# facebookresearch/CODD

Hardware: AMD Instinct MI355X
Metric: frames/sec full CODD forward @960x540 (whole job) (higher is better)
Workload: dtype f32 (split-bf16 MFMA operands, f32 accumulate; HITNet + context network + Fusion exact f32); 1 GPU; full CODD (HITNetMF + Motion/RAFT3D iters=16 + Fusion) 960x540 padded to 960x576, max_disp=320, one video per GPU, steady-state frames (idx>=1), synthetic stereo sequence, random-init weights; conv_precision=split, hip_graph=True, frames_per_gpu=304, prewarm_frames=150, side_streams=True, library=codd_amd/csrc/libcodd_hip.so, full=False

## Files before the change

codd_amd/_abi.py:

```python
import ctypes as C
import os

from . import build as _build

c_float_p = C.POINTER(C.c_float)


class View(C.Structure):
    _fields_ = [("ptr", C.c_void_p), ("ctot", C.c_int), ("coff", C.c_int)]


class XsView(C.Structure):
    _fields_ = [("ptr", C.c_void_p), ("c8", C.c_int), ("hp", C.c_int), ("wp", C.c_int), ("bt", C.c_int),
                ("bl", C.c_int), ("o8", C.c_int), ("terms", C.c_int)]


class ConvParams(C.Structure):
    _fields_ = [
        ("in0", View), ("in1", View), ("C0", C.c_int), ("C1", C.c_int),
        ("B", C.c_int), ("Hin", C.c_int), ("Win", C.c_int),
        ("wpacked", C.c_void_p), ("bias", C.c_void_p),
        ("res1", View), ("res2", View), ("post", View),
        ("out", C.c_void_p), ("out_ctot", C.c_int), ("out_coff", C.c_int),
        ("Cout", C.c_int), ("Hout", C.c_int), ("Wout", C.c_int),
# ... 8 lines not shown
    ]


ACT = dict(none=0, lrelu=1, relu=2, sigmoid=3, tanh=4, mish=5, relu_ch0=6)




class RollParams(C.Structure):
    _fields_ = [("in0", View), ("in1", View), ("C0", C.c_int), ("C1", C.c_int),
                ("B", C.c_int), ("H", C.c_int), ("W", C.c_int), ("C", C.c_int), ("mode", C.c_int),
                ("wA", C.c_void_p), ("bA", C.c_void_p), ("wB", C.c_void_p), ("bB", C.c_void_p),
                ("actA", C.c_int), ("actB", C.c_int), ("residual", C.c_int),
                ("out", C.c_void_p), ("out_ctot", C.c_int), ("out_coff", C.c_int), ("cout_store", C.c_int),
                ("rh", C.c_int)]


_i, _f, _p, _ll = C.c_int, C.c_float, C.c_void_p, C.c_longlong

SIGNATURES = {
    "codd_abi_version": (_i, []),
    "codd_conv2d": (_i, [C.POINTER(ConvParams), _p]),
    "codd_conv2d_check": (_i, [C.POINTER(ConvParams)]),
    "codd_conv2d_multi": (_i, [C.POINTER(ConvParams), _i, _p]),
    "codd_roll_packed_size": (_ll, [_i, _i, _i]),
    "codd_roll_pack_weights": (_i, [_p, _p, _i, _i, _i, _i, _p]),
    "codd_conv_roll": (_i, [C.POINTER(RollParams), _p]),
    "codd_conv2d_packed_size": (_ll, [_i] * 6),
    "codd_conv2d_pack_weights": (_i, [_p, _p, _i, _i, _i, _i, _i, _i, _p]),
    "codd_tile_costvol_argmin": (_i, [_p, _p, _i, _i, _i, _i, _i, _i, _p, _i, _i, _p, _i, _i, _i, _p]),
    "codd_tile_warp_cost": (_i, [_p, _p, _i, _i, _i, _i, View, View, _i, _p, _p, _p]),
    "codd_hyp_upsample": (_i, [View, _i, _i, _i, _f, _p, _i, _i, _p]),
    "codd_hyp_select": (_i, [_p, View, View, _i, _i, _i, _p, _i, _i, _p]),
    "codd_instnorm": (_i, [_p, _i, _i, _i, _p, _p, _i, _p, _p]),
    "codd_instnorm_xs": (_i, [_p, _i, _i, _i, _i, _p, _p, _i, _i, _p, XsView, _p]),
    "codd_conv2d_pack_weights_ex": (_i, [_p, _p, _i, _i, _i, _i, _i, _i, _ll, _ll, _f, _p]),
    "codd_allpairs_corr": (_i, [_p, _p, _i, _i, _i, _i, _p, _p, _p, _p, _p, _p]),
    "codd_allpairs_corr_scratch": (_ll, [_i, _i, _i, _i]),
    "codd_avgpool2": (_i, [_p, _i, _i, _i, _p, _p]),
    "codd_induced_flow": (_i, [_p, _p, _i, _i, _i, _f, _f, _f, _f, _p, _p]),
    "codd_context_split": (_i, [_p, _i, _i, _p, _p, _p]),
    "codd_se3_identity": (_i, [_p, _ll, _p]),
    "codd_corr_lookup": (_i, [_p, _p, _p, _p, _p, _i, _i, _i, _i, _p, _p]),
    "codd_raft_geometry": (_i, [_p, _p, _p, _i, _i, _i, _f, _f, _f, _f, _p, _p, _p]),
    "codd_se3_gn_step": (_i, [_p, _p, _i, _p, _p, _p, _p, _i, _i, _i, _f, _f, _f, _f, _i, _f, _f, _p, _p]),
    "codd_se3_gn_scratch": (_ll, [_i, _i, _i, _i]),
    "codd_set_option": (_i, [_i, _i]),
    "codd_get_option": (_i, [_i]),
    "codd_se3_gn_step_heads": (_i, [_p, XsView, _p, _p, _p, _p, _i, _i, _i, _f, _f, _f, _f, _i, _f, _f, _p, _p, _p]),
    "codd_cvx_upsample": (_i, [_p, _p, _i, _i, _i, _i, _i, _p, _p]),
    "codd_cvx_upsample_se3_weight": (_i, [_p, _p, _p, _i, _i, _i, _p, _p, _p]),
    "codd_disp_to_depth": (_i, [_p, _ll, _f, _p, _p]),
    "codd_subsample": (_i, [_p, _i, _i, _i, _i, _i, _i, _p, _p]),
    "codd_splat": (_i, [_p, _p, _i, _i, _i, _i, _i, _p, _i, _p, _i, _i, _i, _i, _i, _f, _f, _f, _f, _f, _f,
                        _p, _p, _p, _p]),
    "codd_splat_scratch": (_ll, [_i, _i, _i, _f]),
    "codd_resize_bilinear": (_i, [_p, _i, _i, _i, _i, _i, _i, _i, _p, _i, _i, _i, _i, _p]),
    "codd_resize_bilinear_add": (_i, [_p, _i, _i, _i, _i, _i, _i, _i, _p, _i, _i, _i, _i, _p, _p]),
    "codd_add_relu": (_i, [_p, _p, _ll, _i, _p, _p]),
    "codd_copy_many": (_i, [_p, _p, _p, _i, _p]),
    "codd_copy": (_i, [_p, _p, _ll, _p]),
    "codd_timestamp": (_i, [_p, _p]),
    "codd_gru_gate_zr": (_i, [_p, _p, _p, _p, _p, _p, _i, _i, _p, _p, _p]),
    "codd_gru_gate_q": (_i, [_p, _p, _p, _p, _p, _p, _p, _i, _i, _p, _p]),
    "codd_gru_gate_zr_xs": (_i, [_p, _p, _p, _p, _p, _p, _i, _i, _i, _p, XsView, _p]),
    "codd_gru_gate_q_xs": (_i, [_p, _p, _p, _p, _p, _p, _p, _i, _i, _i, _p, XsView, _p]),
# ... 98 lines not shown
```

codd_amd/csrc/stereo.hip:

```cpp
#include "common.h"
#include <stdlib.h>

#define CV_TPB 16
__global__ __launch_bounds__(256) void costvol_argmin_kernel(const float* __restrict__ L, const float* __restrict__ R,
                                                             int C, int Ht, int Wt, int Wr, int D, float* cost,
                                                             int cost_ctot, int cost_coff, float* disp, int disp_ctot,
                                                             int disp_coff, int zero_dxdy) {
  extern __shared__ float sm[];
  const int tid = threadIdx.x, lane = tid & 63, wave = tid >> 6;
  const int xt0 = blockIdx.x * CV_TPB, y = blockIdx.y, b = blockIdx.z;
  const int win = D + 4 * (CV_TPB - 1);
  const int base = 4 * xt0 - (D - 1);
  float* rl = sm;
  float* ll = sm + C * win;
  const float* Rb = R + ((size_t)b * C * Ht + y) * Wr;
  for (int e = tid; e < C * win; e += 256) {
    const int c = e / win, i = e - c * win, gx = base + i;
    rl[e] = (gx >= 0 && gx < Wr) ? Rb[(size_t)c * Ht * Wr + gx] : 0.f;
  }
  const float* Lb = L + ((size_t)b * C * Ht + y) * Wt;
  for (int e = tid; e < C * CV_TPB; e += 256) {
    const int c = e / CV_TPB, i = e - c * CV_TPB, gx = xt0 + i;
    ll[e] = gx < Wt ? Lb[(size_t)c * Ht * Wt + gx] : 0.f;
  }
// ... 105 lines not shown
  }
}

extern "C" int codd_tile_costvol_argmin(const float* L, const float* R, int B, int C, int Ht, int Wt, int Wr, int D,
                                        float* cost, int cost_ctot, int cost_coff, float* disp, int disp_ctot,
                                        int disp_coff, int zero_dxdy, void* stream) {
  if (!L || !R || !cost || !disp || B < 1 || C < 1 || D < 1 || Ht < 1 || Wt < 1) return CODD_EINVAL;
  hipStream_t st = (hipStream_t)stream;
  if ((D & 3) == 0) {
    int tpb = 16;
    for (;; tpb >>= 1) {
      const int win = D + 4 * (tpb - 1);
      const size_t lds = (size_t)(C * win + C * tpb) * sizeof(float);
      if (lds > 64 * 1024) { if (tpb == 16) return CODD_EUNSUPPORTED; continue; }
      dim3 grid(cdiv(Wt, tpb), Ht, B);
#define CV_LAUNCH(T) costvol_argmin4_kernel<T><<<grid, 256, lds, st>>>(L, R, C, Ht, Wt, Wr, D, cost, cost_ctot, cost_coff, disp, disp_ctot, disp_coff, zero_dxdy)
      if (tpb == 64) CV_LAUNCH(64); else if (tpb == 32) CV_LAUNCH(32); else CV_LAUNCH(16);
#undef CV_LAUNCH
      break;
    }
    CODD_LAUNCH_CHECK();
    return CODD_OK;
  }
  const int win = D + 4 * (CV_TPB - 1);
  size_t lds = (size_t)(C * win + C * CV_TPB) * sizeof(float);
  if (lds > 64 * 1024) return CODD_EUNSUPPORTED;
  dim3 grid(cdiv(Wt, CV_TPB), Ht, B);
  costvol_argmin_kernel<<<grid, 256, lds, st>>>(L, R, C, Ht, Wt, Wr, D, cost, cost_ctot, cost_coff,
                                                disp, disp_ctot, disp_coff, zero_dxdy);
  CODD_LAUNCH_CHECK();
  return CODD_OK;
}

template <bool STAGE>
__global__ __launch_bounds__(256) void tile_warp_kernel(const float* __restrict__ fl, const float* __restrict__ fr,
                                                        int C, int Ht, int Wt, codd_view h0, codd_view h1, int nhyp,
                                                        float* out0, float* out1) {
  extern __shared__ __attribute__((aligned(16))) float srow[];
  const int txr = blockIdx.x * blockDim.x + threadIdx.x;
  const int yy = blockIdx.y;
  const int b = blockIdx.z;
  if (!STAGE && txr >= Wt) return;
  const bool live = txr < Wt;
  const int tx = live ? txr : Wt - 1;
  const int ty = yy >> 2, iy = yy & 3;
  const int H = 4 * Ht, W = 4 * Wt;
  if (STAGE) {
    const float4* src = (const float4*)(fr + (size_t)b * C * H * W + (size_t)yy * W);
    const int w4 = W >> 2, chw4 = (H * W) >> 2;
    for (int c = 0; c < C; ++c)
      for (int x4 = threadIdx.x; x4 < w4; x4 += blockDim.x) ((float4*)srow)[c * w4 + x4] = src[(size_t)c * chw4 + x4];
    __syncthreads();
  }
  const size_t thw = (size_t)Ht * Wt, tpix = (size_t)ty * Wt + tx;
  const float* flb = fl + (size_t)b * C * H * W + (size_t)yy * W + 4 * tx;
  const float* frb = fr + (size_t)b * C * H * W + (size_t)yy * W;
  const size_t chw = (size_t)H * W;

  int f0[2][4];
  float a[2][4];
  unsigned okm[2] = {0u, 0u};
#pragma unroll
  for (int hsel = 0; hsel < 2; ++hsel) {
    const codd_view hv = (hsel && nhyp == 2) ? h1 : h0;
    const float* hp = hv.ptr + ((size_t)b * hv.ctot + hv.coff) * thw + tpix;
    const float d = hp[0], dx = hp[thw], dy = hp[2 * thw];
#pragma unroll
    for (int ix = 0; ix < 4; ++ix) {
      const float delta = d + (ix - 1.5f) * dx + (iy - 1.5f) * dy;
      const float xs = (float)(4 * tx + ix) - delta;
      const float fl0 = floorf(xs);
      a[hsel][ix] = xs - fl0;
      f0[hsel][ix] = (int)fminf(fmaxf(fl0, -4.f), (float)W + 4.f);
#pragma unroll
      for (int q = 0; q < 4; ++q)
        if ((unsigned)(f0[hsel][ix] - 1 + q) < (unsigned)W) okm[hsel] |= 1u << (ix * 4 + q);
    }
  }
  float fea[4] = {0.f, 0.f, 0.f, 0.f};
  float cv[2][3][4] = {{{0.f}}};
#pragma unroll 2
  for (int c = 0; c < C; ++c) {
    const float4 l4 = *(const float4*)(flb + c * chw);
    const float lv[4] = {l4.x, l4.y, l4.z, l4.w};
    const float* rr = frb + c * chw;
    float t[2][4][4];
#pragma unroll
    for (int hsel = 0; hsel < 2; ++hsel) {
      if (hsel < nhyp) {
#pragma unroll
        for (int ix = 0; ix < 4; ++ix)
#pragma unroll
          for (int q = 0; q < 4; ++q) {
            const int xi = min(max(f0[hsel][ix] - 1 + q, 0), W - 1);
            t[hsel][ix][q] = STAGE ? srow[c * W + xi] : rr[xi];
          }
      }
    }
#pragma unroll
    for (int ix = 0; ix < 4; ++ix) fea[ix] += fabsf(lv[ix]);
#pragma unroll
    for (int hsel = 0; hsel < 2; ++hsel) {
      if (hsel < nhyp) {
#pragma unroll
        for (int ix = 0; ix < 4; ++ix) {
          float tq[4];
#pragma unroll
          for (int q = 0; q < 4; ++q) tq[q] = (okm[hsel] >> (ix * 4 + q)) & 1u ? t[hsel][ix][q] : 0.f;
          const float w1 = a[hsel][ix], w0 = 1.f - a[hsel][ix];
          cv[hsel][0][ix] += fabsf(lv[ix] - (w0 * tq[2] + w1 * tq[3]));
          cv[hsel][1][ix] += fabsf(lv[ix] - (w0 * tq[1] + w1 * tq[2]));
          cv[hsel][2][ix] += fabsf(lv[ix] - (w0 * tq[0] + w1 * tq[1]));
        }
      }
    }
  }
  if (!live) return;
#pragma unroll
  for (int ix = 0; ix < 4; ++ix) {
    const int ch = iy * 4 + ix;
    const size_t o = (size_t)b * 64 * thw + tpix;
    out0[o + (size_t)ch * thw] = fea[ix];
    if (nhyp == 2) out1[o + (size_t)ch * thw] = fea[ix];
#pragma unroll
    for (int k = 0; k < 3; ++k) {
      out0[o + (size_t)(16 + k * 16 + ch) * thw] = cv[0][k][ix];
      if (nhyp == 2) out1[o + (size_t)(16 + k * 16 + ch) * thw] = cv[1][k][ix];
    }
  }
}

extern "C" int codd_tile_warp_cost(const float* fl, const float* fr, int B, int C, int Ht, int Wt, codd_view hyp0,
                                   codd_view hyp1, int nhyp, float* out0, float* out1, void* stream) {
  if (!fl || !fr || !hyp0.ptr || !out0 || nhyp < 1 || nhyp > 2 || (nhyp == 2 && (!hyp1.ptr || !out1)))
    return CODD_EINVAL;
  const size_t lds = (size_t)C * 4 * Wt * sizeof(float);
  if (lds <= 96 * 1024 && ((uintptr_t)fr & 15) == 0) {
    if (lds > 64 * 1024 &&
        hipFuncSetAttribute((const void*)tile_warp_kernel<true>, hipFuncAttributeMaxDynamicSharedMemorySize, (int)lds) != hipSuccess)
      return CODD_EUNSUPPORTED;
    const int bx = Wt > 128 ? 256 : (Wt > 64 ? 128 : 64);
    dim3 grid(cdiv(Wt, bx), 4 * Ht, B);
    tile_warp_kernel<true><<<grid, bx, lds, (hipStream_t)stream>>>(fl, fr, C, Ht, Wt, hyp0, hyp1, nhyp, out0, out1);
    CODD_LAUNCH_CHECK();
    return CODD_OK;
  }
  const int bx = 64;
  dim3 grid(cdiv(Wt, bx), 4 * Ht, B);
  tile_warp_kernel<false><<<grid, bx, 0, (hipStream_t)stream>>>(fl, fr, C, Ht, Wt, hyp0, hyp1, nhyp, out0, out1);
  CODD_LAUNCH_CHECK();
  return CODD_OK;
}

__global__ void hyp_upsample_kernel(codd_view in, int h, int w, float scale, float* out, int out_ctot, int out_coff,
                                    long long total) {
  long long e = (long long)blockIdx.x * blockDim.x + threadIdx.x;
  if (e >= total) return;
  const int W2 = 2 * w, H2 = 2 * h;
  const int x = (int)(e % W2);
  long long t = e / W2;
  const int y = (int)(t % H2); t /= H2;
  const int c = (int)(t % 16);
  const int b = (int)(t / 16);
  const size_t hw = (size_t)h * w;
  const float* ip = in.ptr + ((size_t)b * in.ctot + in.coff) * hw + (size_t)(y >> 1) * w + (x >> 1);
  float v;
  if (c == 0) {
    const float cx = (x & 1) ? 0.5f : -0.5f, cy = (y & 1) ? 0.5f : -0.5f;
    v = (ip[0] + cx * ip[hw] + cy * ip[2 * hw]) * scale;
  } else {
    v = ip[(size_t)c * hw];
  }
  out[((size_t)b * out_ctot + out_coff + c) * (size_t)(4 * hw) + (size_t)y * W2 + x] = v;
}

extern "C" int codd_hyp_upsample(codd_view in, int B, int h, int w, float scale, float* out, int out_ctot,
                                 int out_coff, void* stream) {
  if (!in.ptr || !out) return CODD_EINVAL;
  long long total = (long long)B * 16 * 4 * h * w;
  hyp_upsample_kernel<<<cdiv(total, 256), 256, 0, (hipStream_t)stream>>>(in, h, w, scale, out, out_ctot, out_coff,
                                                                         total);
  CODD_LAUNCH_CHECK();
  return CODD_OK;
}

__global__ void hyp_select_kernel(const float* __restrict__ upd, codd_view cur, codd_view prev, int hw, float* out,
                                  int out_ctot, int out_coff, long long total) {
  long long e = (long long)blockIdx.x * blockDim.x + threadIdx.x;
  if (e >= total) return;
  const int pix = (int)(e % hw);
  long long t = e / hw;
  const int c = (int)(t % 16);
  const int b = (int)(t / 16);
  const float* u = upd + (size_t)b * 34 * hw + pix;
  const bool sel_cur = u[hw] > u[0];
  float v;
  if (sel_cur) v = cur.ptr[((size_t)b * cur.ctot + cur.coff + c) * hw + pix] + u[(size_t)(18 + c) * hw];
  else v = prev.ptr[((size_t)b * prev.ctot + prev.coff + c) * hw + pix] + u[(size_t)(2 + c) * hw];
  if (c == 0) v = fmaxf(v, 0.f);
  out[((size_t)b * out_ctot + out_coff + c) * hw + pix] = v;
}

extern "C" int codd_hyp_select(const float* upd, codd_view cur, codd_view prev, int B, int h, int w, float* out,
                               int out_ctot, int out_coff, void* stream) {
  if (!upd || !cur.ptr || !prev.ptr || !out) return CODD_EINVAL;
  long long total = (long long)B * 16 * h * w;
  hyp_select_kernel<<<cdiv(total, 256), 256, 0, (hipStream_t)stream>>>(upd, cur, prev, h * w, out, out_ctot, out_coff,
                                                                       total);
  CODD_LAUNCH_CHECK();
  return CODD_OK;
}

extern "C" int codd_abi_version(void) { return CODD_ABI_VERSION; }

static int g_opt[CODD_OPT_COUNT] = {192, 5};
int codd_opt(int key) { return g_opt[key]; }
extern "C" int codd_get_option(int key) { return key >= 0 && key < CODD_OPT_COUNT ? g_opt[key] : CODD_EINVAL; }
extern "C" int codd_set_option(int key, int value) {
  if (key < 0 || key >= CODD_OPT_COUNT) return CODD_EINVAL;
  if (key == CODD_OPT_GN_Q4 && (value < 16 || value > 4096)) return CODD_EINVAL;
  if (key == CODD_OPT_GN_BUILDER && value != 3 && value != 5) return CODD_EINVAL;
  const int prev = g_opt[key];
  g_opt[key] = value;
  return prev;
}
```

codd_amd/ops.py:

```python
import collections
import ctypes as C

import torch

from . import _abi
from ._abi import ACT, ConvParams, View


class RuntimeState:
    _RUNTIME_KEYS = ("_side", "_pending", "_nowait", "_fk", "_xs", "_runners", "_kside", "_h4c", "_ctx4c", "_fused_now", "_pipe")

    def __getstate__(self):
        state = self.__dict__.copy()
        for k in self._RUNTIME_KEYS:
            state.pop(k, None)
        return state


class Slice:
    __slots__ = ("buf", "coff", "c")

    def __init__(self, buf, coff=0, c=None):
        assert buf.is_contiguous() and buf.dtype == torch.float32
        self.buf, self.coff = buf, coff
# ... 901 lines not shown


def tile_warp_cost(fl, fr, hyp0, hyp1=None):
    lib = _abi.load()
    _require_gpu(fl)
    B, Cc, H, W = fl.shape
    Ht, Wt = H // 4, W // 4
    out0 = torch.empty(B, 64, Ht, Wt, device=fl.device, dtype=torch.float32)
    out1 = torch.empty_like(out0) if hyp1 is not None else None
    _abi.check(lib.codd_tile_warp_cost(fl.data_ptr(), fr.data_ptr(), B, Cc, Ht, Wt, _view(hyp0), _view(hyp1),
                                       2 if hyp1 is not None else 1, out0.data_ptr(),
                                       None if out1 is None else out1.data_ptr(), _stream()), "tile_warp_cost")
    return out0, out1


def hyp_upsample(h, scale, out):
    lib = _abi.load()
    hs, os_ = _as_slice(h), _as_slice(out)
    B, _, hh, ww = hs.shape
    _abi.check(lib.codd_hyp_upsample(_view(hs), B, hh, ww, float(scale), os_.buf.data_ptr(), os_.buf.shape[1],
                                     os_.coff, _stream()), "hyp_upsample")
    return out


def hyp_select(upd, cur, prev, out):
    lib = _abi.load()
    B, _, hh, ww = upd.shape
    os_ = _as_slice(out)
    _abi.check(lib.codd_hyp_select(upd.data_ptr(), _view(cur), _view(prev), B, hh, ww, os_.buf.data_ptr(),
                                   os_.buf.shape[1], os_.coff, _stream()), "hyp_select")
    return out


def _f32(*shape, like):
    return torch.empty(*shape, device=like.device, dtype=torch.float32)


def instnorm(x, relu=True, res=None, res_relu=False, xs_out=None, want_fp32=True):
    lib = _abi.load()
    _require_gpu(x)
    B, Cc, H, W = x.shape
    stats = _f32(128 * B * Cc, like=x)
    if xs_out is not None:
        assert (xs_out.B, xs_out.H, xs_out.W) == (B, H, W) and Cc % 8 == 0 and Cc <= 8 * xs_out.c8
        y = torch.empty_like(x) if want_fp32 else None
        _abi.check(lib.codd_instnorm_xs(x.data_ptr(), B, Cc, H, W, stats.data_ptr(), _ptr(res), int(relu), int(res_relu),
                                        _ptr(y), _xs_view(xs_out), _stream()), "instnorm_xs")
        return y
    assert not res_relu
    y = torch.empty_like(x)
    _abi.check(lib.codd_instnorm(x.data_ptr(), B, Cc, H * W, stats.data_ptr(),
                                 None if res is None else res.data_ptr(), int(relu), y.data_ptr(), _stream()),
               "instnorm")
    return y


_ALLPAIRS_CFGS = ((2, 8, 32, 4, 2, 4, 2, 3, 1), (1, 16, 32, 4, 2, 4, 2, 3, 1), (1, 16, 32, 4, 2, 4, 1, 3, 1), (1, 12, 32, 4, 2, 4, 2, 3, 1),
                  (1, 12, 32, 4, 2, 4, 1, 3, 1), (1, 10, 32, 4, 2, 2, 2, 3, 1), (2, 8, 32, 4, 2, 4, 1, 3, 1),
                  (1, 8, 32, 2, 2, 4, 1, 3, 1), (1, 8, 16, 2, 2, 4, 1, 3, 1))
_ALLPAIRS_PICK = {}


def allpairs_corr_split(f1, f2):
    lib = _abi.load()
    _require_gpu(f1)
    B, D, h, w = f1.shape
# ... 612 lines not shown
```

codd_amd/stereo.py:

```python

import torch
import torch.nn as nn

from . import ops
from .ops import Slice
from .registry import MODELS, build_backbone, build_loss, register


def _lrelu():
    return nn.LeakyReLU(0.2, inplace=True)


def packed(m, deconv=False, cout_keep=None):
    ver = (m.weight.data_ptr(), m.weight._version, None if m.bias is None else m.bias._version)
    cache = m.__dict__.setdefault("_codd_packed", {})
    ent = cache.get(cout_keep)
    if ent is None or ent[0] != ver:
        ent = cache[cout_keep] = (ver, ops.PackedConv(m.weight, m.bias, deconv, cout_keep))
    return ent[1]


def invalidate_packed(module):
    for m in module.modules():
        m.__dict__.pop("_codd_packed", None)
# ... 150 lines not shown
            if fk is None or fk.dev != fea_l[0].device:
                fk = self.__dict__["_fk"] = ops.Fork(fea_l[0].device, n - 1)
            hyps = [fk.run(lvl, level, lvl) for lvl in range(n - 1)] + [level(n - 1)]
            fk.join()
        else:
            hyps = [level(lvl) for lvl in range(n)]
        return [None, hyps]


def _convbn(i, o, k, s, p, d):
    return nn.Sequential(nn.Conv2d(i, o, k, s, d if d > 1 else p, d))


class BasicBlock(nn.Module):

    def __init__(self, c1, c2, s, downsample, p, d):
        super().__init__()
        self.conv1 = nn.Sequential(_convbn(c1, c2, 3, s, p, d), _lrelu())
        self.conv2 = _convbn(c2, c2, 3, 1, p, d)

    def run(self, x):
        c1, c2 = self.conv1[0][0], self.conv2[0]
        same3 = all(c.kernel_size == (3, 3) and c.stride == (1, 1) and c.padding == (1, 1) and c.dilation == (1, 1) for c in (c1, c2))
        if same3 and ops.use_roll(c1.out_channels, *x.shape) and c1.in_channels == c1.out_channels:
            return ops.conv_roll(x, roll(self, "block", [(c1, "lrelu"), (c2, "lrelu")], residual=True))
        t = cv(c1, x, act="lrelu")
        return cv(c2, t, res1=x, act="lrelu")


def _resblock(c, d=1):
    return nn.Sequential(BasicBlock(c, c, s=1, p=1, downsample=None, d=d), _lrelu())


class TileUpdate0(nn.Module):

    def __init__(self, in_c, out_c, hid_c):
        super().__init__()
        self.decrease = nn.Sequential(nn.Conv2d(64, 16, 1), _lrelu())
        self.conv0 = nn.Sequential(nn.Conv2d(in_c, hid_c, 1), _lrelu())
        self.resblock0 = _resblock(32)
        self.resblock1 = _resblock(32)
        self.lastconv = nn.Conv2d(hid_c, out_c, 3, 1, 1)

    def forward(self, fl, fr, hyp):
        aug = hyp.buf
        w, _ = ops.tile_warp_cost(fl, fr, hyp)
        cv(self.decrease[0], w, act="lrelu", out=Slice(aug, 16, 16))
        t = cv(self.conv0[0], aug, act="lrelu")
        t = self.resblock0[0].run(t)
        t = self.resblock1[0].run(t)
        return [cv(self.lastconv, t, res1=hyp, act="relu_ch0")]


class TileUpdate(nn.Module):

    def __init__(self):
        super().__init__()
        self.decrease = nn.Sequential(nn.Conv2d(64, 16, 1), _lrelu())
        self.conv0 = nn.Sequential(nn.Conv2d(64, 32, 1), _lrelu())
        self.resblock0 = _resblock(32)
        self.resblock1 = _resblock(32)
        self.lastconv = nn.Conv2d(32, 34, 3, 1, 1)

    def forward(self, fl, fr, hyp, prev):
        aug = hyp.buf
        up = Slice(aug, 32, 16)
        ops.hyp_upsample(prev, 2.0, up)
        w0, w1 = ops.tile_warp_cost(fl, fr, hyp, up)
        with ops.deferred_convs():
            cv(self.decrease[0], w0, act="lrelu", out=Slice(aug, 16, 16))
            cv(self.decrease[0], w1, act="lrelu", out=Slice(aug, 48, 16))
        t = cv(self.conv0[0], aug, act="lrelu")
        t = self.resblock0[0].run(t)
        t = self.resblock1[0].run(t)
        upd = cv(self.lastconv, t)
        B, _, h, w = upd.shape
        out = torch.empty(B, 16, h, w, device=upd.device, dtype=torch.float32)
        return [ops.hyp_select(upd, hyp, up, out)]


class PostTileUpdate(nn.Module):

    def __init__(self, in_c, out_c, hid_c, resblk_num, final=False):
        super().__init__()
        self.conv1 = nn.Sequential(nn.Conv2d(in_c, hid_c, 1), _lrelu(), nn.Conv2d(hid_c, hid_c, 3, 1, 1), _lrelu())
        self.resblocks = nn.Sequential(*[_resblock(hid_c, 3 if (i == 1 and not final) else 1)
                                         for i in range(resblk_num)])
        self.lastconv = nn.Conv2d(hid_c, out_c, 3, padding=1)
        self._final = final

    def forward(self, fl, prev):
        if ops.use_roll(self.conv1[0].out_channels, *fl.shape):
            t = ops.conv_roll(fl, roll(self, "head", [(self.conv1[0], "lrelu"), (self.conv1[2], "lrelu")]), x2=prev)
        else:
            t = cv(self.conv1[0], fl, x2=prev, act="lrelu")
            t = cv(self.conv1[2], t, act="lrelu")
        for blk in self.resblocks:
            t = blk[0].run(t)
        if self._final:
            return ops.conv2d(t, packed(self.lastconv, cout_keep=1), pad=1, res1=Slice(_buf(prev), _off(prev), 1),
                              act="relu")
        return cv(self.lastconv, t, res1=prev, act="relu_ch0")




class FinalTileUpdate(PostTileUpdate):

    def __init__(self, in_c, out_c, hid_c, resblk_num):
        super().__init__(in_c, out_c, hid_c, resblk_num, final=True)


def _buf(x):
    return x.buf if isinstance(x, Slice) else x


def _off(x):
    return x.coff if isinstance(x, Slice) else 0


def _up1(h):
    B, _, hh, ww = h.shape
    out = torch.empty(B, 16, 2 * hh, 2 * ww, device=h.device, dtype=torch.float32)
    return ops.hyp_upsample(h, 1.0, out)


@register
class TilePropagation(nn.Module):

    def __init__(self):
        super().__init__()
        self.tile_update0 = TileUpdate0(32, 16, 32)
        self.tile_update1 = TileUpdate()
        self.tile_update2 = TileUpdate()
        self.tile_update3 = TileUpdate()
        self.tile_update4 = TileUpdate()
        self.tile_update4_1 = PostTileUpdate(40, 16, 32, 4)
        self.tile_update5 = PostTileUpdate(32, 16, 32, 4)
        self.tile_update6 = FinalTileUpdate(32, 3, 16, 2)

    def forward(self, fea_l, fea_r, init):
        h = self.tile_update0(fea_l[0], fea_r[0], init[0])[0]
        for i, upd in enumerate((self.tile_update1, self.tile_update2, self.tile_update3, self.tile_update4), 1):
            h = upd(fea_l[i], fea_r[i], init[i], h)[0]
        r1 = self.tile_update4_1(fea_l[2], h)
        r05 = self.tile_update5(fea_l[3], _up1(r1))
        return self.tile_update6(fea_l[4], _up1(r05))


@register
class HITNetMF(ops.RuntimeState, nn.Module):

    def __init__(self, backbone, initialization, propagation, loss=None):
        super().__init__()
        self.backbone = build_backbone(backbone)
        self.tile_init = MODELS.build(initialization)
        self.tile_update = MODELS.build(propagation)
        self.freezed = False
        self.loss = build_loss(loss) if loss is not None else None

    def extract_feat(self, img):
        return self.backbone(img)

    def _stereo_matching_pipelined(self, left_img, right_img):
        B, dev = left_img.shape[0], left_img.device
        ti, tu = self.tile_init, self.tile_update
        g = self.backbone.stages(ops.batch_pair(left_img, right_img))
        feas = [next(g), next(g)]
        L, R = (lambda i: feas[i][:B]), (lambda i: feas[i][B:])
# ... 47 lines not shown
```

include/codd_hip.h:

```cpp
#ifndef CODD_HIP_H
#define CODD_HIP_H

#ifdef __cplusplus
extern "C" {
#endif

#define CODD_ABI_VERSION 12

#define CODD_OK 0
#define CODD_EINVAL (-1)
#define CODD_EUNSUPPORTED (-2)

enum { CODD_OPT_GN_Q4 = 0, CODD_OPT_GN_BUILDER = 1, CODD_OPT_COUNT = 2 };
int codd_set_option(int key, int value);
int codd_get_option(int key);

enum { CODD_ACT_NONE = 0, CODD_ACT_LRELU02 = 1, CODD_ACT_RELU = 2, CODD_ACT_SIGMOID = 3,
       CODD_ACT_TANH = 4, CODD_ACT_MISH = 5, CODD_ACT_RELU_CH0 = 6 };

typedef struct {
  const float* ptr;
  int ctot;
  int coff;
} codd_view;
// ... 68 lines not shown
  codd_view in0, in1;
  int C0, C1;
  int B, H, W;
  int C;
  int mode;
  const float* wA;
  const float* bA;
  const float* wB;
  const float* bB;
  int actA, actB;
  int residual;
  float* out;
  int out_ctot, out_coff, cout_store;
  int rh;
} codd_roll_params;
long long codd_roll_packed_size(int C, int k, int Cin);
int codd_roll_pack_weights(const float* w, float* packed, int C, int Cout, int Cin, int k, void* stream);
int codd_conv_roll(const codd_roll_params* p, void* stream);

int codd_tile_costvol_argmin(const float* L, const float* R, int B, int C, int Ht, int Wt, int Wr, int D,
                             float* cost, int cost_ctot, int cost_coff,
                             float* disp, int disp_ctot, int disp_coff, int zero_dxdy, void* stream);

int codd_tile_warp_cost(const float* fl, const float* fr, int B, int C, int Ht, int Wt,
                        codd_view hyp0, codd_view hyp1, int nhyp,
                        float* out0, float* out1, void* stream);

int codd_hyp_upsample(codd_view in, int B, int h, int w, float scale,
                      float* out, int out_ctot, int out_coff, void* stream);

int codd_hyp_select(const float* upd, codd_view cur, codd_view prev, int B, int h, int w,
                    float* out, int out_ctot, int out_coff, void* stream);

int codd_instnorm(const float* x, int B, int C, int HW, float* stats, const float* res, int relu,
                  float* y, void* stream);
int codd_instnorm_xs(const float* x, int B, int C, int H, int W, float* stats, const float* res, int relu,
                     int relu_after_res, float* y, codd_xs_view xs, void* stream);

int codd_allpairs_corr(const float* f1, const float* f2, int B, int D, int h, int w,
                       float* lvl0, float* lvl1, float* lvl2, float* lvl3, float* scratch, void* stream);
long long codd_allpairs_corr_scratch(int B, int D, int h, int w);
int codd_avgpool2(const float* in, int BC, int h, int w, float* out, void* stream);

int codd_corr_lookup(const float* lvl0, const float* lvl1, const float* lvl2, const float* lvl3,
                     const float* coords, int cstride, int B, int h, int w, float* out, void* stream);

int codd_raft_geometry(const float* T, const float* depth1, const float* depth2, int B, int h, int w,
                       float fx, float fy, float cx, float cy, float* xyz, float* minfo, void* stream);

long long codd_se3_gn_scratch(int B, int h, int w, int radius);
int codd_se3_gn_step(float* T, const float* ae, int ae_c, const float* xyz, const float* delta,
                     const float* weight, const float* depth1, int B, int h, int w,
                     float fx, float fy, float cx, float cy, int radius, float lm, float ep,
                     float* Hb, void* stream);

int codd_se3_gn_step_heads(float* T, codd_xs_view hidden, const void* head_w, const float* head_b,
                           const float* xyz, const float* depth1, int B, int h, int w, float fx, float fy,
                           float cx, float cy, int radius, float lm, float ep, float* weight_out, float* Hb,
                           void* stream);

int codd_cvx_upsample(const float* data, const float* mask, int B, int h, int w, int dim, int mode,
                      float* out, void* stream);
int codd_cvx_upsample_se3_weight(const float* T, const float* weight, const float* mask, int B, int h, int w,
                                 float* T_out, float* weight_out, void* stream);

int codd_disp_to_depth(const float* disp, long long n, float bf, float* depth, void* stream);
// ... 123 lines not shown
```

Baseline: 104.3 frames/s.

## Fuse tile warp cost, hypothesis upsample/select and 1x1 decrease conv into one kernel

Adds a tile_update_head kernel that, per tile block, stages left and right feature rows in LDS, computes the warp cost features for one or two hypotheses, and applies the 1x1 decrease conv with MFMA, writing straight into the aug buffer. For TileUpdate levels it also folds the previous level's hyp_select and hyp_upsample into the same kernel by passing a deferred HypTriple. This removes several launches and the round trip of intermediate warp/cost tensors through global memory. In exchange it uses much larger LDS and 1024-thread blocks (possible occupancy loss), adds a slow fallback path for taps outside the staged window, and changes FMA contraction order in the shared warp helpers.

```diff
diff --git a/codd_amd/_abi.py b/codd_amd/_abi.py
--- a/codd_amd/_abi.py
+++ b/codd_amd/_abi.py
@@ -64,6 +64,7 @@
     "codd_tile_warp_cost": (_i, [_p, _p, _i, _i, _i, _i, View, View, _i, _p, _p, _p]),
     "codd_hyp_upsample": (_i, [View, _i, _i, _i, _f, _p, _i, _i, _p]),
     "codd_hyp_select": (_i, [_p, View, View, _i, _i, _i, _p, _i, _i, _p]),
+    "codd_tile_update_head": (_i, [_p, _p, _i, _i, _i, _i, View, _i, View, _p, View, _p, _p, _i, _p, _i, _i, _i, _p]),
     "codd_instnorm": (_i, [_p, _i, _i, _i, _p, _p, _i, _p, _p]),
     "codd_instnorm_xs": (_i, [_p, _i, _i, _i, _i, _p, _p, _i, _i, _p, XsView, _p]),
     "codd_conv2d_pack_weights_ex": (_i, [_p, _p, _i, _i, _i, _i, _i, _i, _ll, _ll, _f, _p]),
diff --git a/codd_amd/csrc/stereo.hip b/codd_amd/csrc/stereo.hip
--- a/codd_amd/csrc/stereo.hip
+++ b/codd_amd/csrc/stereo.hip
@@ -161,6 +161,63 @@
   return CODD_OK;
 }
 
+__device__ __forceinline__ unsigned warp_tap(float d, float dx, float dy, int tx, int iy, int ix, int W, int& f0,
+                                             float& a) {
+#pragma clang fp contract(off)
+  const float delta = __builtin_fmaf(dx, ix - 1.5f, d) + (iy - 1.5f) * dy;
+  const float xs = (float)(4 * tx + ix) - delta;
+  const float fl0 = floorf(xs);
+  a = xs - fl0;
+  f0 = (int)fminf(fmaxf(fl0, -4.f), (float)W + 4.f);
+  unsigned ok = 0u;
+#pragma unroll
+  for (int q = 0; q < 4; ++q)
+    if ((unsigned)(f0 - 1 + q) < (unsigned)W) ok |= 1u << q;
+  return ok;
+}
+
+__device__ __forceinline__ unsigned warp_taps(float d, float dx, float dy, int tx, int iy, int W, int (&f0)[4],
+                                              float (&a)[4]) {
+  unsigned okm = 0u;
+#pragma unroll
+  for (int ix = 0; ix < 4; ++ix) okm |= warp_tap(d, dx, dy, tx, iy, ix, W, f0[ix], a[ix]) << (ix * 4);
+  return okm;
+}
+
+__device__ __forceinline__ void warp_accumulate_ix(float lv, const float (&t)[4], unsigned ok, float a, float& cv0,
+                                                   float& cv1, float& cv2) {
+#pragma clang fp contract(off)
+  float tq[4];
+#pragma unroll
+  for (int q = 0; q < 4; ++q) tq[q] = (ok >> q) & 1u ? t[q] : 0.f;
+  const float w1 = a, w0 = 1.f - a;
+  cv0 += fabsf(lv - __builtin_fmaf(w1, tq[3], w0 * tq[2]));
+  cv1 += fabsf(lv - __builtin_fmaf(w1, tq[2], w0 * tq[1]));
+  cv2 += fabsf(lv - __builtin_fmaf(w1, tq[1], w0 * tq[0]));
+}
+
+__device__ __forceinline__ void warp_accumulate(const float (&lv)[4], const float (&t)[4][4], unsigned okm,
+                                                const float (&a)[4], float (&cv)[3][4]) {
+#pragma unroll
+  for (int ix = 0; ix < 4; ++ix)
+    warp_accumulate_ix(lv[ix], t[ix], (okm >> (ix * 4)) & 15u, a[ix], cv[0][ix], cv[1][ix], cv[2][ix]);
+}
+
+__device__ __forceinline__ float hyp_upsample_d(float d, float dx, float dy, int x, int y, float scale) {
+  const float cx = (x & 1) ? 0.5f : -0.5f, cy = (y & 1) ? 0.5f : -0.5f;
+  return (d + cx * dx + cy * dy) * scale;
+}
+
+__device__ __forceinline__ bool hyp_select_cur(const float* u, size_t hw) { return u[hw] > u[0]; }
+__device__ __forceinline__ float hyp_select_value(const float* u, bool sel_cur, const codd_view& cur,
+                                                  const codd_view& prev, int b, int c, size_t hw, size_t pix) {
+  float v;
+  if (sel_cur) v = cur.ptr[((size_t)b * cur.ctot + cur.coff + c) * hw + pix] + u[(size_t)(18 + c) * hw];
+  else v = prev.ptr[((size_t)b * prev.ctot + prev.coff + c) * hw + pix] + u[(size_t)(2 + c) * hw];
+  if (c == 0) v = fmaxf(v, 0.f);
+  return v;
+}
+
 template <bool STAGE>
 __global__ __launch_bounds__(256) void tile_warp_kernel(const float* __restrict__ fl, const float* __restrict__ fr,
                                                         int C, int Ht, int Wt, codd_view h0, codd_view h1, int nhyp,
@@ -194,17 +251,7 @@
     const codd_view hv = (hsel && nhyp == 2) ? h1 : h0;
     const float* hp = hv.ptr + ((size_t)b * hv.ctot + hv.coff) * thw + tpix;
     const float d = hp[0], dx = hp[thw], dy = hp[2 * thw];
-#pragma unroll
-    for (int ix = 0; ix < 4; ++ix) {
-      const float delta = d + (ix - 1.5f) * dx + (iy - 1.5f) * dy;
-      const float xs = (float)(4 * tx + ix) - delta;
-      const float fl0 = floorf(xs);
-      a[hsel][ix] = xs - fl0;
-      f0[hsel][ix] = (int)fminf(fmaxf(fl0, -4.f), (float)W + 4.f);
-#pragma unroll
-      for (int q = 0; q < 4; ++q)
-        if ((unsigned)(f0[hsel][ix] - 1 + q) < (unsigned)W) okm[hsel] |= 1u << (ix * 4 + q);
-    }
+    okm[hsel] = warp_taps(d, dx, dy, tx, iy, W, f0[hsel], a[hsel]);
   }
   float fea[4] = {0.f, 0.f, 0.f, 0.f};
   float cv[2][3][4] = {{{0.f}}};
@@ -229,20 +276,8 @@
 #pragma unroll
     for (int ix = 0; ix < 4; ++ix) fea[ix] += fabsf(lv[ix]);
 #pragma unroll
-    for (int hsel = 0; hsel < 2; ++hsel) {
-      if (hsel < nhyp) {
-#pragma unroll
-        for (int ix = 0; ix < 4; ++ix) {
-          float tq[4];
-#pragma unroll
-          for (int q = 0; q < 4; ++q) tq[q] = (okm[hsel] >> (ix * 4 + q)) & 1u ? t[hsel][ix][q] : 0.f;
-          const float w1 = a[hsel][ix], w0 = 1.f - a[hsel][ix];
-          cv[hsel][0][ix] += fabsf(lv[ix] - (w0 * tq[2] + w1 * tq[3]));
-          cv[hsel][1][ix] += fabsf(lv[ix] - (w0 * tq[1] + w1 * tq[2]));
-          cv[hsel][2][ix] += fabsf(lv[ix] - (w0 * tq[0] + w1 * tq[1]));
-        }
-      }
-    }
+    for (int hsel = 0; hsel < 2; ++hsel)
+      if (hsel < nhyp) warp_accumulate(lv, t[hsel], okm[hsel], a[hsel], cv[hsel]);
   }
   if (!live) return;
 #pragma unroll
@@ -295,8 +330,7 @@
   const float* ip = in.ptr + ((size_t)b * in.ctot + in.coff) * hw + (size_t)(y >> 1) * w + (x >> 1);
   float v;
   if (c == 0) {
-    const float cx = (x & 1) ? 0.5f : -0.5f, cy = (y & 1) ? 0.5f : -0.5f;
-    v = (ip[0] + cx * ip[hw] + cy * ip[2 * hw]) * scale;
+    v = hyp_upsample_d(ip[0], ip[hw], ip[2 * hw], x, y, scale);
   } else {
     v = ip[(size_t)c * hw];
   }
@@ -322,11 +356,7 @@
   const int c = (int)(t % 16);
   const int b = (int)(t / 16);
   const float* u = upd + (size_t)b * 34 * hw + pix;
-  const bool sel_cur = u[hw] > u[0];
-  float v;
-  if (sel_cur) v = cur.ptr[((size_t)b * cur.ctot + cur.coff + c) * hw + pix] + u[(size_t)(18 + c) * hw];
-  else v = prev.ptr[((size_t)b * prev.ctot + prev.coff + c) * hw + pix] + u[(size_t)(2 + c) * hw];
-  if (c == 0) v = fmaxf(v, 0.f);
+  const float v = hyp_select_value(u, hyp_select_cur(u, hw), cur, prev, b, c, hw, pix);
   out[((size_t)b * out_ctot + out_coff + c) * hw + pix] = v;
 }
 
@@ -336,6 +366,223 @@
   long long total = (long long)B * 16 * h * w;
   hyp_select_kernel<<<cdiv(total, 256), 256, 0, (hipStream_t)stream>>>(upd, cur, prev, h * w, out, out_ctot, out_coff,
                                                                        total);
+  CODD_LAUNCH_CHECK();
+  return CODD_OK;
+}
+
+struct TileHeadK {
+  const float* fl; const float* fr;
+  int C, Ht, Wt;
+  codd_view hyp;
+  int prev_mode;
+  codd_view prev, pcur;
+  const float* upd;
+  const float* wquad; const float* bias;
+  int act;
+  float* aug; int aug_ctot;
+  int tw, tw_shift, winw, reach;
+  int lgl, lgr;
+};
+
+constexpr int HEAD_STAGE_DEPTH = 6;
+
+template <int NH, bool FAST>
+__device__ __forceinline__ void head_channels(int C, const float* sl, int ls, const float* sr, int rs, const float* rg,
+                                              size_t chw, int xw0, int xw1, const int (&f0)[NH], const float (&a)[NH],
+                                              const unsigned (&okm)[NH], const unsigned (&inw)[NH], float& fea,
+                                              float (&cv)[NH][3]) {
+  constexpr int UNROLL = FAST ? 4 : 1;
+#pragma unroll UNROLL
+  for (int c = 0; c < C; ++c) {
+    const float lv = sl[c * ls];
+    const float* rl = sr + c * rs;
+    float tp[NH][4];
+#pragma unroll
+    for (int hs = 0; hs < NH; ++hs)
+#pragma unroll
+      for (int q = 0; q < 4; ++q) {
+        const int xi = f0[hs] - 1 + q;
+        const float v = rl[min(max(xi, xw0), xw1)];
+        tp[hs][q] = FAST || ((inw[hs] >> q) & 1u) ? v : rg[(size_t)c * chw + xi];
+      }
+    fea += fabsf(lv);
+#pragma unroll
+    for (int hs = 0; hs < NH; ++hs) warp_accumulate_ix(lv, tp[hs], okm[hs], a[hs], cv[hs][0], cv[hs][1], cv[hs][2]);
+  }
+}
+
+template <int NH>
+__global__ __launch_bounds__(1024) void tile_update_head_kernel(const TileHeadK k) {
+  extern __shared__ __attribute__((aligned(16))) float smem[];
+  const int TW = k.tw, NT = 16 * TW;
+  const int tid = threadIdx.x, ix = tid & 3, t = (tid >> 2) & (TW - 1), iy = tid >> (k.tw_shift + 2);
+  const int tx0 = blockIdx.x * TW, ty = blockIdx.y, b = blockIdx.z;
+  const int C = k.C, Ht = k.Ht, Wt = k.Wt, H = 4 * Ht, W = 4 * Wt;
+  const bool live = tx0 + t < Wt;
+  const int tx = live ? tx0 + t : Wt - 1;
+  const int lw = min(4 * TW, W - 4 * tx0), LW = 4 * TW, winw = k.winw;
+  const int xw0 = min(max(4 * tx0 - k.reach, 0), W - winw);
+  float* sl = smem;
+  float* sr = smem + C * 4 * LW;
+  const size_t chw = (size_t)H * W;
+  const float* flb = k.fl + (size_t)b * C * chw + (size_t)(4 * ty) * W;
+  const float* frb = k.fr + (size_t)b * C * chw + (size_t)(4 * ty) * W;
+
+  {
+    const int lw4 = lw >> 2, ww4 = winw >> 2, nl = (C * 4) << k.lgl, nu = nl + ((C * 4) << k.lgr);
+    for (int u0 = tid; u0 < nu; u0 += HEAD_STAGE_DEPTH * NT) {
+      float4 v[HEAD_STAGE_DEPTH];
+      int dst[HEAD_STAGE_DEPTH];
+#pragma unroll
+      for (int i = 0; i < HEAD_STAGE_DEPTH; ++i) {
+        const int u = u0 + i * NT;
+        const bool left = u < nl;
+        const int e = left ? u : u - nl, lg = left ? k.lgl : k.lgr;
+        const int cr = e >> lg, x4 = e & ((1 << lg) - 1);
+        const bool on = u < nu && x4 < (left ? lw4 : ww4);
+        const float* src = (left ? flb + 4 * tx0 : frb + xw0) + (size_t)(cr >> 2) * chw + (cr & 3) * W + 4 * x4;
+        dst[i] = on ? (left ? cr * LW : C * 4 * LW + cr * winw) + 4 * x4 : -1;
+        v[i] = *(const float4*)(on ? src : flb);
+      }
+#pragma unroll
+      for (int i = 0; i < HEAD_STAGE_DEPTH; ++i)
+        if (dst[i] >= 0) *(float4*)(smem + dst[i]) = v[i];
+    }
+  }
+  const int lane = tid & 63, wave = tid >> 6, g = lane >> 4, j = lane & 15;
+  const int ngrp = TW >> 4, njobs = NH * ngrp, nwaves = NT >> 6;
+  float4 wreg[4];
+  if (wave < njobs) {
+#pragma unroll
+    for (int gr = 0; gr < 4; ++gr) wreg[gr] = ((const float4*)k.wquad)[(4 * gr + g) * 16 + j];
+  }
+
+  const size_t thw = (size_t)Ht * Wt, tpix = (size_t)ty * Wt + tx;
+  int f0[NH];
+  float a[NH];
+  unsigned okm[NH], inw[NH];
+  {
+    const float* hp = k.hyp.ptr + ((size_t)b * k.hyp.ctot + k.hyp.coff) * thw + tpix;
+    okm[0] = warp_tap(hp[0], hp[thw], hp[2 * thw], tx, iy, ix, W, f0[0], a[0]);
+  }
+  if (NH == 2) {
+    const int h = (Ht + 1) >> 1, w = (Wt + 1) >> 1, cm = 4 * iy + ix;
+    const size_t hw = (size_t)h * w, cp = (size_t)(ty >> 1) * w + (tx >> 1);
+    const float* u = k.upd + (size_t)b * 34 * hw + cp;
+    const bool sel_cur = k.prev_mode == 2 ? hyp_select_cur(u, hw) : false;
+    float s[3];
+#pragma unroll
+    for (int c = 0; c < 3; ++c)
+      s[c] = k.prev_mode == 2 ? hyp_select_value(u, sel_cur, k.pcur, k.prev, b, c, hw, cp)
+                              : k.prev.ptr[((size_t)b * k.prev.ctot + k.prev.coff + c) * hw + cp];
+    float mine = k.prev_mode == 2 ? hyp_select_value(u, sel_cur, k.pcur, k.prev, b, cm, hw, cp)
+                                  : k.prev.ptr[((size_t)b * k.prev.ctot + k.prev.coff + cm) * hw + cp];
+    float d = hyp_upsample_d(s[0], s[1], s[2], tx, ty, 2.0f);
+    asm volatile("" : "+v"(d));
+    if (cm == 0) mine = d;
+    if (live) k.aug[((size_t)b * k.aug_ctot + 32 + cm) * thw + tpix] = mine;
+    okm[NH - 1] = warp_tap(d, s[1], s[2], tx, iy, ix, W, f0[NH - 1], a[NH - 1]);
+  }
+  const int xw1 = xw0 + winw - 1;
+  bool fast = true;
+#pragma unroll
+  for (int hs = 0; hs < NH; ++hs) {
+    inw[hs] = ~okm[hs] & 15u;
+#pragma unroll
+    for (int q = 0; q < 4; ++q)
+      if ((unsigned)(f0[hs] - 1 + q - xw0) < (unsigned)winw) inw[hs] |= 1u << q;
+    fast = fast && inw[hs] == 15u;
+  }
+  __syncthreads();
+
+  float fea = 0.f;
+  float cv[NH][3];
+#pragma unroll
+  for (int hs = 0; hs < NH; ++hs)
+#pragma unroll
+    for (int kk = 0; kk < 3; ++kk) cv[hs][kk] = 0.f;
+  const float* slt = sl + iy * LW + 4 * (tx - tx0) + ix;
+  const float* srt = sr + iy * winw - xw0;
+  const float* frt = frb + iy * W;
+  if (fast) head_channels<NH, true>(C, slt, 4 * LW, srt, 4 * winw, frt, chw, xw0, xw1, f0, a, okm, inw, fea, cv);
+  else head_channels<NH, false>(C, slt, 4 * LW, srt, 4 * winw, frt, chw, xw0, xw1, f0, a, okm, inw, fea, cv);
+  __syncthreads();
+
+#pragma unroll
+  for (int hs = 0; hs < NH; ++hs) {
+    smem[((hs * 16 + iy) * TW + t) * 4 + ix] = fea;
+#pragma unroll
+    for (int kk = 0; kk < 3; ++kk) smem[((hs * 16 + (kk + 1) * 4 + iy) * TW + t) * 4 + ix] = cv[hs][kk];
+  }
+  __syncthreads();
+
+  const float4* img = (const float4*)smem;
+  if (wave < njobs) {
+    const int hs = wave / ngrp, grp = wave - hs * ngrp;
+    const float4* ip = img + (hs * 16 + g) * TW + 16 * grp + j;
+    f32x4 acc = (f32x4){0.f, 0.f, 0.f, 0.f};
+#pragma unroll
+    for (int gr = 0; gr < 4; ++gr) {
+      const float4 av = wreg[gr], bv = ip[4 * gr * TW];
+      acc = __builtin_amdgcn_mfma_f32_16x16x4f32(av.x, bv.x, acc, 0, 0, 0);
+      acc = __builtin_amdgcn_mfma_f32_16x16x4f32(av.y, bv.y, acc, 0, 0, 0);
+      acc = __builtin_amdgcn_mfma_f32_16x16x4f32(av.z, bv.z, acc, 0, 0, 0);
+      acc = __builtin_amdgcn_mfma_f32_16x16x4f32(av.w, bv.w, acc, 0, 0, 0);
+    }
+    const int ox = tx0 + 16 * grp + j;
+    if (ox < Wt) {
+#pragma unroll
+      for (int r = 0; r < 4; ++r) {
+        const int co = 4 * g + r;
+        float v = acc[r];
+        if (k.bias) v += k.bias[co];
+        v = act_apply(v, k.act, co);
+        k.aug[((size_t)b * k.aug_ctot + 16 + 32 * hs + co) * thw + (size_t)ty * Wt + ox] = v;
+      }
+    }
+  }
+  (void)nwaves;
+}
+
+extern "C" int codd_tile_update_head(const float* fl, const float* fr, int B, int C, int Ht, int Wt, codd_view hyp,
+                                     int prev_mode, codd_view prev, const float* upd, codd_view pcur,
+                                     const float* wquad, const float* bias, int act, float* aug, int aug_ctot,
+                                     int reach, int tiles, void* stream) {
+  if (!fl || !fr || !hyp.ptr || !wquad || !aug || prev_mode < 0 || prev_mode > 2 || (prev_mode >= 1 && !prev.ptr) ||
+      (prev_mode == 2 && (!upd || !pcur.ptr)) || B < 1 || C < 1 || Ht < 1 || Wt < 1 || reach < 0 ||
+      !(tiles == 0 || tiles == 16 || tiles == 32 || tiles == 64))
+    return CODD_EINVAL;
+  const int nh = prev_mode ? 2 : 1;
+  if (aug_ctot < 32 * nh || (((uintptr_t)fl | (uintptr_t)fr | (uintptr_t)wquad) & 15) != 0 || Ht > 65535 || B > 65535 ||
+      Wt > (1 << 24))
+    return CODD_EUNSUPPORTED;
+  const int W = 4 * Wt;
+  TileHeadK k;
+  k.fl = fl; k.fr = fr; k.C = C; k.Ht = Ht; k.Wt = Wt; k.hyp = hyp; k.prev_mode = prev_mode; k.prev = prev; k.pcur = pcur;
+  k.upd = upd; k.wquad = wquad; k.bias = bias; k.act = act; k.aug = aug; k.aug_ctot = aug_ctot;
+  k.reach = (int)(((long long)(reach < W ? reach : W) + 3) & ~3LL);
+  size_t lds = 0;
+  int tw = Wt > 32 ? 64 : (Wt > 16 ? 32 : 16);
+  while (!tiles && tw > 16 && (long long)cdiv(Wt, tw) * Ht * B < 128) tw >>= 1;
+  if (tiles && tiles < tw) tw = tiles;
+  for (;; tw >>= 1) {
+    if (tw < 16) return CODD_EUNSUPPORTED;
+    k.winw = 4 * tw + k.reach + 4 < W ? 4 * tw + k.reach + 4 : W;
+    lds = (size_t)4 * C * (4 * tw + k.winw) * sizeof(float);
+    if (lds <= 160 * 1024) break;
+  }
+  const size_t image = (size_t)nh * 64 * tw * sizeof(float);
+  if (lds < image) lds = image;
+  k.tw = tw;
+  k.tw_shift = tw == 64 ? 6 : (tw == 32 ? 5 : 4);
+  k.lgl = k.tw_shift;
+  for (k.lgr = 0; (1 << k.lgr) < (k.winw >> 2); ++k.lgr) {}
+  const void* fn = nh == 2 ? (const void*)tile_update_head_kernel<2> : (const void*)tile_update_head_kernel<1>;
+  if (lds > 64 * 1024 && hipFuncSetAttribute(fn, hipFuncAttributeMaxDynamicSharedMemorySize, (int)lds) != hipSuccess)
+    return CODD_EUNSUPPORTED;
+  dim3 grid(cdiv(Wt, tw), Ht, B);
+  if (nh == 2) tile_update_head_kernel<2><<<grid, 16 * tw, lds, (hipStream_t)stream>>>(k);
+  else tile_update_head_kernel<1><<<grid, 16 * tw, lds, (hipStream_t)stream>>>(k);
   CODD_LAUNCH_CHECK();
   return CODD_OK;
 }
diff --git a/codd_amd/ops.py b/codd_amd/ops.py
--- a/codd_amd/ops.py
+++ b/codd_amd/ops.py
@@ -957,6 +957,71 @@
     return out
 
 
+class HypTriple:
+    __slots__ = ("upd", "cur", "up")
+
+    def __init__(self, upd, cur, up):
+        self.upd, self.cur, self.up = upd, cur, up
+
+    @property
+    def shape(self):
+        B, _, h, w = self.upd.shape
+        return (B, 16, h, w)
+
+    def materialise(self):
+        B, _, h, w = self.upd.shape
+        out = torch.empty(B, 16, h, w, device=self.upd.device, dtype=torch.float32)
+        return hyp_select(self.upd, self.cur, self.up, out)
+
+
+def resolved_conv_cfg(pc, B, Hout, Wout):
+    terms = _TERMS.get(CONV_PRECISION, 0)
+    cfg = pc.tuned.get(_plain_key(B, Hout, Wout, terms))
+    return None if cfg is None else decode_cfg(cfg, pc.mb, terms)
+
+
+def _plain_key(B, Hout, Wout, terms):
+    return (Hout, Wout, B, 1, 1, 1, 1, 0, False, terms) + (("co",) if _CORESIDENT and terms else ())
+
+
+def pin_conv_cfg(pc, B, Hout, Wout, cfg):
+    pc.tuned[_plain_key(B, Hout, Wout, _TERMS.get(CONV_PRECISION, 0))] = tuple(cfg)
+
+
+def tile_head_cfg(pc, B, Ht, Wt):
+    f = resolved_conv_cfg(pc, B, Ht, Wt)
+    ok = (f is not None and f.layout == 1 and f.mb == 1 and (pc.cout_eff, pc.cin, pc.kh, pc.kw) == (16, 64, 1, 1)
+          and not pc.deconv)
+    return f if ok else None
+
+
+def _launch_tile_head(lib, args):
+    return lib.codd_tile_update_head(*args)
+
+
+def tile_update_head(fl, fr, hyp, pc, cfg, prev=None, act="lrelu", reach=None, tiles=0):
+    lib = _abi.load()
+    _require_gpu(fl)
+    B, Cc, H, W = fl.shape
+    Ht, Wt = H // 4, W // 4
+    hs = _as_slice(hyp)
+    aug = hs.buf
+    assert fl.is_contiguous() and fr.is_contiguous() and fr.shape == fl.shape and aug.shape[2:] == (Ht, Wt)
+    mode, pv, upd, pcur = 0, None, None, None
+    if isinstance(prev, HypTriple):
+        mode, pv, upd, pcur = 2, prev.up, prev.upd, prev.cur
+        assert upd.is_contiguous() and tuple(upd.shape) == (B, 34, (Ht + 1) // 2, (Wt + 1) // 2)
+    elif prev is not None:
+        mode, pv = 1, prev
+        assert tuple(_as_slice(prev).shape) == (B, 16, (Ht + 1) // 2, (Wt + 1) // 2)
+    wq = pc.packed(cfg.ck, 1, 1)
+    _abi.check(_launch_tile_head(lib, (
+        fl.data_ptr(), fr.data_ptr(), B, Cc, Ht, Wt, _view(hs), mode, _view(pv), None if upd is None else upd.data_ptr(),
+        _view(pcur), wq.data_ptr(), None if pc.bias is None else pc.bias.data_ptr(), ACT[act], aug.data_ptr(),
+        aug.shape[1], W // 5 + 8 if reach is None else reach, tiles, _stream())), "tile_update_head")
+    return Slice(aug, 32, 16) if mode else None
+
+
 def _f32(*shape, like):
     return torch.empty(*shape, device=like.device, dtype=torch.float32)
 
diff --git a/codd_amd/stereo.py b/codd_amd/stereo.py
--- a/codd_amd/stereo.py
+++ b/codd_amd/stereo.py
@@ -206,6 +206,17 @@
     return nn.Sequential(BasicBlock(c, c, s=1, p=1, downsample=None, d=d), _lrelu())
 
 
+FUSE_TILE_HEAD = True
+FUSE_TILE_HEAD_MAX_TILES = 16384
+
+
+def _head_cfg(decrease, fl):
+    B, _, H, W = fl.shape
+    if not FUSE_TILE_HEAD or (H // 4) * (W // 4) > FUSE_TILE_HEAD_MAX_TILES:
+        return None
+    return ops.tile_head_cfg(packed(decrease), B, H // 4, W // 4)
+
+
 class TileUpdate0(nn.Module):
 
     def __init__(self, in_c, out_c, hid_c):
@@ -218,8 +229,12 @@
 
     def forward(self, fl, fr, hyp):
         aug = hyp.buf
-        w, _ = ops.tile_warp_cost(fl, fr, hyp)
-        cv(self.decrease[0], w, act="lrelu", out=Slice(aug, 16, 16))
+        cfg = _head_cfg(self.decrease[0], fl)
+        if cfg is not None:
+            ops.tile_update_head(fl, fr, hyp, packed(self.decrease[0]), cfg)
+        else:
+            w, _ = ops.tile_warp_cost(fl, fr, hyp)
+            cv(self.decrease[0], w, act="lrelu", out=Slice(aug, 16, 16))
         t = cv(self.conv0[0], aug, act="lrelu")
         t = self.resblock0[0].run(t)
         t = self.resblock1[0].run(t)
@@ -236,21 +251,28 @@
         self.resblock1 = _resblock(32)
         self.lastconv = nn.Conv2d(32, 34, 3, 1, 1)
 
+    select_later = False
+
     def forward(self, fl, fr, hyp, prev):
         aug = hyp.buf
         up = Slice(aug, 32, 16)
-        ops.hyp_upsample(prev, 2.0, up)
-        w0, w1 = ops.tile_warp_cost(fl, fr, hyp, up)
-        with ops.deferred_convs():
-            cv(self.decrease[0], w0, act="lrelu", out=Slice(aug, 16, 16))
-            cv(self.decrease[0], w1, act="lrelu", out=Slice(aug, 48, 16))
+        cfg = _head_cfg(self.decrease[0], fl)
+        if cfg is not None:
+            ops.tile_update_head(fl, fr, hyp, packed(self.decrease[0]), cfg, prev=prev)
+        else:
+            if isinstance(prev, ops.HypTriple):
+                prev = prev.materialise()
+            ops.hyp_upsample(prev, 2.0, up)
+            w0, w1 = ops.tile_warp_cost(fl, fr, hyp, up)
+            with ops.deferred_convs():
+                cv(self.decrease[0], w0, act="lrelu", out=Slice(aug, 16, 16))
+                cv(self.decrease[0], w1, act="lrelu", out=Slice(aug, 48, 16))
         t = cv(self.conv0[0], aug, act="lrelu")
         t = self.resblock0[0].run(t)
         t = self.resblock1[0].run(t)
         upd = cv(self.lastconv, t)
-        B, _, h, w = upd.shape
-        out = torch.empty(B, 16, h, w, device=upd.device, dtype=torch.float32)
-        return [ops.hyp_select(upd, hyp, up, out)]
+        sel = ops.HypTriple(upd, hyp, up)
+        return [sel if FUSE_TILE_HEAD and self.select_later else sel.materialise()]
 
 
 class PostTileUpdate(nn.Module):
@@ -309,6 +331,8 @@
         self.tile_update2 = TileUpdate()
         self.tile_update3 = TileUpdate()
         self.tile_update4 = TileUpdate()
+        for m in (self.tile_update1, self.tile_update2, self.tile_update3):
+            m.select_later = True
         self.tile_update4_1 = PostTileUpdate(40, 16, 32, 4)
         self.tile_update5 = PostTileUpdate(32, 16, 32, 4)
         self.tile_update6 = FinalTileUpdate(32, 3, 16, 2)
diff --git a/include/codd_hip.h b/include/codd_hip.h
--- a/include/codd_hip.h
+++ b/include/codd_hip.h
@@ -124,6 +124,11 @@
 int codd_hyp_select(const float* upd, codd_view cur, codd_view prev, int B, int h, int w,
                     float* out, int out_ctot, int out_coff, void* stream);
 
+int codd_tile_update_head(const float* fl, const float* fr, int B, int C, int Ht, int Wt, codd_view hyp,
+                          int prev_mode, codd_view prev, const float* upd, codd_view pcur,
+                          const float* wquad, const float* bias, int act, float* aug, int aug_ctot,
+                          int reach, int tiles, void* stream);
+
 int codd_instnorm(const float* x, int B, int C, int HW, float* stats, const float* res, int relu,
                   float* y, void* stream);
 int codd_instnorm_xs(const float* x, int B, int C, int H, int W, float* stats, const float* res, int relu,
```

Result: no change. 104.2 frames/s (-0.1%).
